# AegisIK/DistMLIP

Measured on NVIDIA H100. Metric: atoms/sec (energy+forces) CHGNet a-Si r_cut=5A, higher is better.
Workload: dtype f32

## Files before the change

### distmlip_b200/csrc/kernels.cu

```cuda
#include "atomic_virial.cuh"
#include "kernels.cuh"
#include "wgmma.cuh"

#include <algorithm>

namespace b2m {

std::atomic<long long> g_launch_count{0};

__device__ __forceinline__ float sigm(float x) {
  float e, r;
  asm("ex2.approx.ftz.f32 %0, %1;" : "=f"(e) : "f"(x * -1.4426950408889634f));
  asm("rcp.approx.ftz.f32 %0, %1;" : "=f"(r) : "f"(1.f + e));
  return r;
}
__device__ __forceinline__ float silu_f(float x) { return x * sigm(x); }
__device__ __forceinline__ float dsilu_f(float x) {
  float s = sigm(x);
  return s * (1.f + x * (1.f - s));
}

__device__ __forceinline__ uint32_t smem_u32(const void* p) { return (uint32_t)__cvta_generic_to_shared(p); }
__device__ __forceinline__ void mbar_init(uint64_t* bar, uint32_t count) {
  asm volatile("mbarrier.init.shared::cta.b64 [%0], %1;" ::"r"(smem_u32(bar)), "r"(count) : "memory");
}
__device__ __forceinline__ void fence_barrier_init() {
  asm volatile("fence.mbarrier_init.release.cluster;" ::: "memory");
  asm volatile("fence.proxy.async.shared::cta;" ::: "memory");
}
__device__ __forceinline__ void mbar_expect_tx(uint64_t* bar, uint32_t bytes) {
  asm volatile("mbarrier.arrive.expect_tx.shared::cta.b64 _, [%0], %1;" ::"r"(smem_u32(bar)), "r"(bytes) : "memory");
}
__device__ __forceinline__ void bulk_g2s(void* dst_smem, const void* src_gmem, uint32_t bytes, uint64_t* bar) {
  asm volatile("cp.async.bulk.shared::cluster.global.mbarrier::complete_tx::bytes [%0], [%1], %2, [%3];" ::"r"(
                   smem_u32(dst_smem)),
               "l"(src_gmem), "r"(bytes), "r"(smem_u32(bar))
               : "memory");
}
__device__ __forceinline__ void mbar_wait(uint64_t* bar, uint32_t parity) {
  uint32_t ok = 0;
  const uint32_t addr = smem_u32(bar);
  do {
    asm volatile(
        "{\n\t.reg .pred p;\n\tmbarrier.try_wait.parity.shared::cta.b64 p, [%1], %2;\n\tselp.u32 %0, 1, 0, p;\n\t}"
        : "=r"(ok)
        : "r"(addr), "r"(parity)
        : "memory");
  } while (!ok);
}
__device__ __forceinline__ uint32_t stage_parity(int it) { return (uint32_t)(it >> 1) & 1u; }
__device__ __forceinline__ void bulk_g2s_image(float* dst, const float* src, uint32_t bytes, uint64_t* bar) {
  mbar_expect_tx(bar, bytes);
  for (uint32_t o = 0; o < bytes; o += 16384u) bulk_g2s(dst + o / 4, src + o / 4, 16384u, bar);
}

__device__ __forceinline__ float ipowf(float x, int n) {
  float r = 1.f;
  for (int i = 0; i < n; i++) r *= x;
  return r;
}
__device__ __forceinline__ void rbf_env_k(float d, float freq, const RadialParams& rp, float& be, float& dbe) {
  const float invd = 1.f / d;
  const float w = freq / rp.rc;
  float s, c;
  sincosf(d * w, &s, &c);
  const float rbf = rp.norm * s * invd;
  const float drbf = rp.norm * (w * c * invd - s * invd * invd);
  const int p = rp.p;
  const float c1 = -(p + 1) * (p + 2) * 0.5f, c2 = (float)(p * (p + 2)), c3 = -p * (p + 1) * 0.5f;
  const float rho = rbf / rp.rc;
  const float rm1 = ipowf(rho, p - 1);
  const float r0 = rm1 * rho, r1 = r0 * rho, r2 = r1 * rho;
  const float env = 1.f + c1 * r0 + c2 * r1 + c3 * r2;
  const float denv = (c1 * p * rm1 + c2 * (p + 1) * r0 + c3 * (p + 2) * r1) / rp.rc;
  const bool ok = rbf <= rp.rc;
  be = ok ? env * rbf : 0.f;
  dbe = ok ? (env + rbf * denv) * drbf : 0.f;
}

constexpr int AR = 4, AC = 16;
struct Map {
  int branch, rb, cb;
  __device__ __forceinline__ Map() {
    const int tid = threadIdx.x;
    branch = tid >> 7;
    const int lane = tid & 31;
    rb = ((tid & 127) >> 5) * 16 + (lane >> 2);
    cb = 2 * (lane & 3);
  }
  __device__ __forceinline__ int row(int i) const { return 64 * (i >> 1) + rb + 8 * (i & 1); }
  __device__ __forceinline__ int col(int j) const { return 8 * (j >> 1) + cb + (j & 1); }
};

template <int KB>
__device__ __forceinline__ void wg_mma64(const float (&x)[KB][4], uint32_t b_hi, uint32_t b_lo, int bk, bool accumulate,
                                         float (&d)[32]) {
  constexpr uint32_t LBO = 8 * 128;
  uint32_t ah[KB][4], al[KB][4];
#pragma unroll
  for (int ks = 0; ks < KB; ks++)
#pragma unroll
    for (int q = 0; q < 4; q++) {
      ah[ks][q] = tf32_hi_bits(x[ks][q]);
      al[ks][q] = __float_as_uint(x[ks][q] - __uint_as_float(ah[ks][q]));
    }
  const uint32_t koff = (uint32_t)(bk / 4) * LBO;
  acc_fence(d);
  wgmma_fence();
#pragma unroll
  for (int ks = 0; ks < KB; ks++) {
#pragma unroll
    for (int term = 0; term < 3; term++) {
      const uint64_t bd = gmma_desc((term == 2 ? b_lo : b_hi) + koff + ks * 2 * LBO, LBO, 128u);
      wgmma_tf32_n64_rA(d, term == 1 ? al[ks] : ah[ks], bd, (accumulate || ks > 0 || term > 0) ? 1 : 0);
    }
  }
  wgmma_commit();
  wgmma_wait_all();
  acc_fence(d);
}

__device__ __forceinline__ void wg_mm64(const float* At, int lda, int row0, int acol, uint32_t b_hi, uint32_t b_lo,
                                        int bk, bool accumulate, float (&d)[32]) {
  const int lane = threadIdx.x & 31;
  const float* p0 = At + (row0 + ((threadIdx.x & 127) >> 5) * 16 + (lane >> 2)) * lda + acol + 2 * (lane & 3);
  const float* p1 = p0 + 8 * lda;
  float x[8][4];
#pragma unroll
  for (int ks = 0; ks < 8; ks++) {
    const float2 u = *reinterpret_cast<const float2*>(p0 + 8 * ks), v = *reinterpret_cast<const float2*>(p1 + 8 * ks);
    x[ks][0] = u.x, x[ks][1] = v.x, x[ks][2] = u.y, x[ks][3] = v.y;
  }
  wg_mma64(x, b_hi, b_lo, bk, accumulate, d);
}

__device__ __forceinline__ void gemm64(const float* At, int lda, int kofs, const float* Bcan, float (&acc)[AR][AC]) {
  const uint32_t bh = s_u32(Bcan), bl = bh + 4096u * 4u;
#pragma unroll
  for (int h = 0; h < 2; h++) {
    float d[32];
    wg_mm64(At, lda, 64 * h, kofs, bh, bl, 0, false, d);
#pragma unroll
    for (int q = 0; q < 32; q++) acc[2 * h + ((q >> 1) & 1)][2 * (q >> 2) + (q & 1)] = d[q];
  }
}

__device__ __forceinline__ void stage_w(float* Wsm, const float* __restrict__ g, int nfloat4) {
  for (int i = threadIdx.x; i < nfloat4; i += NT) reinterpret_cast<float4*>(Wsm)[i] = reinterpret_cast<const float4*>(g)[i];
  fence_proxy_async_smem();
}

__global__ void k_embed(int n, const int* __restrict__ type, const float* __restrict__ emb, float* __restrict__ x0) {
  const int64_t i = blockIdx.x * (int64_t)blockDim.x + threadIdx.x;
  if (i >= (int64_t)n * 16) return;
  const int r = (int)(i >> 4), c4 = (int)(i & 15);
  reinterpret_cast<float4*>(x0)[(size_t)r * 16 + c4] = reinterpret_cast<const float4*>(emb)[(size_t)type[r] * 16 + c4];
}
void launch_embed(cudaStream_t st, int n, const int* type, const float* emb, float* x0) {
  if (n <= 0) return;
  k_embed<<<cdiv((int64_t)n * 16, 256), 256, 0, st>>>(n, type, emb, x0);
  B2M_CK(cudaGetLastError());
  g_launch_count++;
}

__global__ void __launch_bounds__(256) k_bond_init(int nb, const float4* __restrict__ b_vec, RadialParams rp,
                                                   const float* __restrict__ W, float* __restrict__ out) {
  __shared__ float be_s[32][12];
  __shared__ float Ws[64 * 9];
  const int b0 = blockIdx.x * 32, tid = threadIdx.x;
  for (int i = tid; i < 576; i += 256) Ws[i] = W[i];
  for (int i = tid; i < 32 * 9; i += 256) {
    const int r = i / 9, k = i % 9;
    float be = 0.f, dbe;
    if (b0 + r < nb) rbf_env_k(b_vec[b0 + r].w, rp.freq[k], rp, be, dbe);
    be_s[r][k] = be;
  }
  __syncthreads();
  for (int i = tid; i < 32 * 64; i += 256) {
    const int r = i >> 6, c = i & 63;
    if (b0 + r >= nb) continue;
    float s = 0.f;
#pragma unroll
    for (int k = 0; k < 9; k++) s = fmaf(be_s[r][k], Ws[c * 9 + k], s);
    out[(size_t)(b0 + r) * 64 + c] = s;
  }
}
void launch_bond_init(cudaStream_t st, int nb, const float4* b_vec, RadialParams rp, const float* W, float* out) {
  if (nb <= 0) return;
  k_bond_init<<<cdiv(nb, 32), 256, 0, st>>>(nb, b_vec, rp, W, out);
  B2M_CK(cudaGetLastError());
  g_launch_count++;
}

struct AngleGeom {
  float cos_raw, cc, theta, na, nb;
  float va[3], vb[3];
};
__device__ __forceinline__ AngleGeom angle_geom(const float4 a, const float4 b) {
  AngleGeom g;
  g.va[0] = a.x, g.va[1] = a.y, g.va[2] = a.z;
  g.vb[0] = b.x, g.vb[1] = b.y, g.vb[2] = b.z;
  g.na = sqrtf(a.x * a.x + a.y * a.y + a.z * a.z);
  g.nb = sqrtf(b.x * b.x + b.y * b.y + b.z * b.z);
  g.cos_raw = -(a.x * b.x + a.y * b.y + a.z * b.z) / (g.na * g.nb);
  const float lo = -1.f + 1e-7f, hi = 1.f - 1e-7f;
  g.cc = fminf(fmaxf(g.cos_raw, lo), hi);
  g.theta = acosf(g.cc);
  return g;
}

__global__ void __launch_bounds__(256) k_angle_init(int64_t na, const int* __restrict__ a_in,
                                                    const int* __restrict__ a_out, const float4* __restrict__ b_vec,
                                                    const float* __restrict__ fa, const float* __restrict__ Wae,
                                                    float* __restrict__ ang0) {
  __shared__ float f_s[128][12];
  __shared__ float Ws[64 * 9];
  const int64_t r0 = (int64_t)blockIdx.x * 128;
  const int tid = threadIdx.x;
  for (int i = tid; i < 576; i += 256) Ws[i] = Wae[i];
  if (tid < 128) {
    const int64_t r = r0 + tid;
    if (r < na) {
      const AngleGeom g = angle_geom(b_vec[a_in[r]], b_vec[a_out[r]]);
      const float ipi = 0.318309886183790672f;
      for (int k = 0; k < 5; k++) {
        float s, c;
        sincosf(g.theta * fa[k], &s, &c);
        f_s[tid][2 * k] = c * ipi;
        if (k >= 1) f_s[tid][2 * k - 1] = s * ipi;
      }
    } else {
      for (int k = 0; k < 9; k++) f_s[tid][k] = 0.f;
    }
  }
  __syncthreads();
  for (int i = tid; i < 16 * 128; i += 256) {
    const int cq = i >> 7, r = i & 127;
    if (r0 + r >= na) continue;
    float v[4] = {0.f, 0.f, 0.f, 0.f};
#pragma unroll
    for (int k = 0; k < 9; k++) {
      const float f = f_s[r][k];
#pragma unroll
      for (int j = 0; j < 4; j++) v[j] = fmaf(f, Ws[(4 * cq + j) * 9 + k], v[j]);
    }
    *reinterpret_cast<float4*>(ang0 + (size_t)(r0 + r) * 64 + 4 * cq) = make_float4(v[0], v[1], v[2], v[3]);
  }
}
void launch_angle_init(cudaStream_t st, int64_t na, const int* a_in, const int* a_out, const float4* b_vec,
                       const float* fa, const float* Wae, float* ang0) {
  if (na <= 0) return;
  k_angle_init<<<cdiv(na, 128), 256, 0, st>>>(na, a_in, a_out, b_vec, fa, Wae, ang0);
  B2M_CK(cudaGetLastError());
  g_launch_count++;
}

__global__ void k_silu(int64_t n, const float* __restrict__ pre, float* __restrict__ out) {
  const int64_t i = blockIdx.x * (int64_t)blockDim.x + threadIdx.x;
  if (i < n) out[i] = silu_f(pre[i]);
}
__global__ void k_dsilu_mul(int64_t n, const float* __restrict__ pre, float* __restrict__ g) {
  const int64_t i = blockIdx.x * (int64_t)blockDim.x + threadIdx.x;
  if (i < n) g[i] *= dsilu_f(pre[i]);
}
void launch_silu(cudaStream_t st, int64_t n, const float* pre, float* out) {
  if (n <= 0) return;
  k_silu<<<cdiv(n, 256), 256, 0, st>>>(n, pre, out);
  B2M_CK(cudaGetLastError());
  g_launch_count++;
}
void launch_dsilu_mul(cudaStream_t st, int64_t n, const float* pre, float* g) {
  if (n <= 0) return;
  k_dsilu_mul<<<cdiv(n, 256), 256, 0, st>>>(n, pre, g);
  B2M_CK(cudaGetLastError());
  g_launch_count++;
}
void launch_zero_rows(cudaStream_t st, float* p, int64_t nfloats) {
  if (nfloats > 0) B2M_CK(cudaMemsetAsync(p, 0, nfloats * sizeof(float), st));
}

constexpr int LDE = 136;

struct EdgeRow {
  int src, dst, bond;
  float d;
};
__device__ __forceinline__ EdgeRow edge_row(const AtomConvArgs& a, int64_t e) {
  EdgeRow r{-1, -1, -1, 1.f};
  if (threadIdx.x < TM && e < a.E) {
    r.src = a.e_src[e];
    r.dst = a.e_dst[e];
    r.bond = a.e_bond[e];
    r.d = a.e_vec[e].w;
  }
  return r;
}
__device__ __forceinline__ void issue_gather(const AtomConvArgs& a, int64_t t, const EdgeRow& row, float* buf,
                                             uint64_t* bar, int* s_src, int* s_dst, int* s_bond, float* s_d) {
  const int tid = threadIdx.x;
  if (tid == 0) mbar_expect_tx(bar, (uint32_t)min((int64_t)TM, a.E - t * TM) * 512u);
  if (tid < TM) {
    if (s_src != nullptr) s_src[tid] = row.src;
    s_dst[tid] = row.dst;
    s_bond[tid] = row.bond;
    s_d[tid] = row.d;
    if (row.src >= 0) bulk_g2s(buf + tid * LDE, a.Aproj + (size_t)row.src * D2, 512u, bar);
  }
}
__device__ __forceinline__ void radial_rows(const AtomConvArgs& a, const float* s_d, int nvalid, float* be_s, float* be8,
                                            float* dbe_s, float* dbe8) {
  const int r = threadIdx.x & 127, half = threadIdx.x >> 7;
  const float d = s_d[r];
  const int k0 = half ? 5 : 0, k1 = half ? 9 : 5;
  for (int k = k0; k < k1; k++) {
    float be = 0.f, dbe = 0.f;
    if (r < nvalid) rbf_env_k(d, a.rp.freq[k], a.rp, be, dbe);
    *(k < 8 ? be_s + r * 8 + k : be8 + r) = be;
    if (dbe_s != nullptr) *(k < 8 ? dbe_s + r * 8 + k : dbe8 + r) = dbe;
  }
}
__device__ __forceinline__ float2 ld_f2(const float* p) { return *reinterpret_cast<const float2*>(p); }
__device__ __forceinline__ void st_f2(float* p, float x, float y) { *reinterpret_cast<float2*>(p) = make_float2(x, y); }

__device__ __forceinline__ constexpr int fq(int ii, int j) { return 4 * (j >> 1) + 2 * ii + (j & 1); }

__device__ __forceinline__ void radial_mma(const Map& m, int h, const float* x_s, const float* img, float (&d)[32]) {
  const float2 u = ld_f2(x_s + m.row(2 * h) * 8 + m.cb), v = ld_f2(x_s + m.row(2 * h + 1) * 8 + m.cb);
  const float x[1][4] = {{u.x, v.x, u.y, v.y}};
  uint32_t b = s_u32(img);
  asm volatile("" : "+r"(b));
  wg_mma64(x, b, b + 512u * 4u, 0, false, d);
}

__device__ __forceinline__ void first_layer_half(const AtomConvArgs& a, const Map& m, int h, const float* tile,
                                                 const int* s_dst, const int* s_bond, const float* be_s,
                                                 const float* be8, const float* rad, int nvalid,
                                                 float (&acc)[AR][AC]) {
  const int c0 = 64 * m.branch + m.cb;
  float2 cv[2][AC / 2], qv[2][AC / 2];
  float b8[2];
  bool viaQ[2], ok[2];
#pragma unroll
  for (int ii = 0; ii < 2; ii++) {
    const int r = m.row(2 * h + ii);
    const int dst = s_dst[r], bond = s_bond[r];
    ok[ii] = r < nvalid;
    viaQ[ii] = a.Qproj != nullptr && bond >= 0;
    const float* cp = a.Cproj + (size_t)max(dst, 0) * D2 + c0;
#pragma unroll
    for (int jj = 0; jj < AC / 2; jj++) cv[ii][jj] = dst >= 0 ? __ldg(reinterpret_cast<const float2*>(cp + 8 * jj)) : make_float2(0.f, 0.f);
    if (viaQ[ii]) {
      const float* qp = a.Qproj + (size_t)bond * D2 + c0;
#pragma unroll
      for (int jj = 0; jj < AC / 2; jj++) qv[ii][jj] = __ldg(reinterpret_cast<const float2*>(qp + 8 * jj));
    } else {
#pragma unroll
      for (int jj = 0; jj < AC / 2; jj++) qv[ii][jj] = make_float2(0.f, 0.f);
    }
    b8[ii] = be8[r];
  }
  float d[32];
  radial_mma(m, h, be_s, rad + ATOM_RAD_M + 1024 * m.branch, d);
#pragma unroll
  for (int j = 0; j < AC; j++) {
    const float m8 = rad[ATOM_RAD_M8 + 64 * m.branch + m.col(j)];
#pragma unroll
    for (int ii = 0; ii < 2; ii++) {
      const int r = m.row(2 * h + ii);
      const float x = tile[r * LDE + 64 * m.branch + m.col(j)];
      const float2 c2 = cv[ii][j >> 1], q2 = qv[ii][j >> 1];
      const float t = viaQ[ii] ? ((j & 1) ? q2.y : q2.x) : fmaf(b8[ii], m8, d[fq(ii, j)]);
      acc[2 * h + ii][j] = ok[ii] ? x + ((j & 1) ? c2.y : c2.x) + t : 0.f;
    }
  }
}

__device__ __forceinline__ void wg_mm64_acc(const float (&x)[AR][AC], int h, const float* Bcan, float (&acc)[AR][AC]) {
  float v[8][4];
#pragma unroll
  for (int ks = 0; ks < 8; ks++) {
    v[ks][0] = x[2 * h][2 * ks], v[ks][1] = x[2 * h + 1][2 * ks];
    v[ks][2] = x[2 * h][2 * ks + 1], v[ks][3] = x[2 * h + 1][2 * ks + 1];
  }
  const uint32_t b_hi = s_u32(Bcan);
  float d[32];
  wg_mma64(v, b_hi, b_hi + 4096u * 4u, 0, false, d);
#pragma unroll
  for (int q = 0; q < 32; q++) acc[2 * h + ((q >> 1) & 1)][2 * (q >> 2) + (q & 1)] = d[q];
}

__device__ __forceinline__ float quad_row_sum(const float (&v)[AR]) {
  const int l = threadIdx.x & 3;
  const bool b0 = l & 1, b1 = l & 2;
  float w[2];
#pragma unroll
  for (int h = 0; h < 2; h++)
    w[h] = (b0 ? v[2 * h + 1] : v[2 * h]) + __shfl_xor_sync(0xffffffffu, b0 ? v[2 * h] : v[2 * h + 1], 1);
  return (b1 ? w[1] : w[0]) + __shfl_xor_sync(0xffffffffu, b1 ? w[0] : w[1], 2);
}

__device__ __forceinline__ void red_add_v4(float* p, float4 v) {
  asm volatile("red.global.add.v4.f32 [%0], {%1, %2, %3, %4};" ::"l"(p), "f"(v.x), "f"(v.y), "f"(v.z), "f"(v.w)
               : "memory");
}

__device__ __forceinline__ void seg_add(float* out, int width, int col, int k, const float4& v, int& cur, float4& sum) {
  if (k != cur) {
    if (cur >= 0) red_add_v4(out + (size_t)cur * width + col, sum);
    cur = k;
    sum = make_float4(0.f, 0.f, 0.f, 0.f);
  }
  if (k >= 0) sum.x += v.x, sum.y += v.y, sum.z += v.z, sum.w += v.w;
}

template <int LPR>
__device__ __forceinline__ void scatter_rows(const float* tile, const int* key0, float* out0, const int* key1,
                                             float* out1, const int* gidx, float* gat, const int* sidx = nullptr,
                                             float* sto = nullptr) {
  constexpr int R = TM * LPR / NT, W = 4 * LPR, B = 8;
  static_assert(R % B == 0 && B % 4 == 0, "batches of B rows, their indices read as int4");
  const int q = threadIdx.x % LPR, r0 = threadIdx.x / LPR * R;
  float4 s0 = make_float4(0.f, 0.f, 0.f, 0.f), s1 = s0;
  int c0 = -1, c1 = -1;
#pragma unroll
  for (int b = 0; b < R; b += B) {
    float4 v[B];
    int k0[B], k1[B], kg[B], ks[B];
#pragma unroll
    for (int i = 0; i < B; i++) v[i] = *reinterpret_cast<const float4*>(tile + (r0 + b + i) * LDE + 4 * q);
    auto ld_idx = [&](const int* idx, bool on, int(&k)[B]) {
#pragma unroll
      for (int i = 0; i < B; i += 4) {
        const int4 x = on ? *reinterpret_cast<const int4*>(idx + r0 + b + i) : make_int4(-1, -1, -1, -1);
        k[i] = x.x, k[i + 1] = x.y, k[i + 2] = x.z, k[i + 3] = x.w;
      }
    };
    ld_idx(key0, out0 != nullptr, k0);
    ld_idx(key1, out1 != nullptr, k1);
    ld_idx(gidx, gat != nullptr, kg);
    ld_idx(sidx, sto != nullptr, ks);
#pragma unroll
    for (int i = 0; i < B; i++) {
      if (ks[i] >= 0) *reinterpret_cast<float4*>(sto + (size_t)ks[i] * W + 4 * q) = v[i];
      if (kg[i] >= 0) red_add_v4(gat + (size_t)kg[i] * W + 4 * q, v[i]);
      seg_add(out0, W, 4 * q, k0[i], v[i], c0, s0);
      seg_add(out1, W, 4 * q, k1[i], v[i], c1, s1);
    }
  }
  if (c0 >= 0) red_add_v4(out0 + (size_t)c0 * W + 4 * q, s0);
  if (c1 >= 0) red_add_v4(out1 + (size_t)c1 * W + 4 * q, s1);
}

struct AtomSmemFwd {
  static constexpr int kTile = 32;
  static constexpr int kW = kTile + 2 * TM * LDE;
  static constexpr int kRad = kW + 16384;
  static constexpr int kBe = kRad + ATOM_RAD;
  static constexpr int kBe8 = kBe + TM * 8;
  static constexpr int kB2 = kBe8 + TM;
  static constexpr int kD = kB2 + 128;
  static constexpr int kIdx = kD + 2 * TM;
  static constexpr int kTotal = kIdx + 4 * TM;
  static constexpr size_t bytes = (size_t)kTotal * 4;
};
static_assert(AtomSmemFwd::bytes <= 232448, "atom-conv forward shared memory");
static_assert(AtomSmemFwd::kW % 4 == 0 && AtomSmemFwd::kRad % 4 == 0 && AtomSmemFwd::kBe % 4 == 0,
              "16-byte aligned images and radial rows");

__global__ void __launch_bounds__(NT, 1) k_atomconv_fwd(const AtomConvArgs a) {
  extern __shared__ __align__(128) float smem[];
  uint64_t* mbar = reinterpret_cast<uint64_t*>(smem);
  float* Wsm = smem + AtomSmemFwd::kW;
  float* rad = smem + AtomSmemFwd::kRad;
  float* be_s = smem + AtomSmemFwd::kBe;
  float* be8 = smem + AtomSmemFwd::kBe8;
  float* b2s = smem + AtomSmemFwd::kB2;

  const int tid = threadIdx.x;
  const int64_t ntiles = (a.E + TM - 1) / TM, step = gridDim.x;
  auto tile_of = [&](int s) { return smem + AtomSmemFwd::kTile + s * TM * LDE; };
  auto d_of = [&](int s) { return smem + AtomSmemFwd::kD + s * TM; };
  auto dst_of = [&](int s) { return reinterpret_cast<int*>(smem + AtomSmemFwd::kIdx) + s * TM; };
  auto bond_of = [&](int s) { return reinterpret_cast<int*>(smem + AtomSmemFwd::kIdx) + (2 + s) * TM; };

  if (tid == 0) {
    mbar_init(&mbar[0], 1);
    mbar_init(&mbar[1], 1);
    fence_barrier_init();
  }
  EdgeRow nxt = edge_row(a, (int64_t)blockIdx.x * TM + tid);
  stage_w(Wsm, a.W2can, 4096);
  stage_w(rad, a.radial, ATOM_RAD / 4);
  if (tid < 128) b2s[tid] = a.b2[tid];
  __syncthreads();
  issue_gather(a, blockIdx.x, nxt, tile_of(0), &mbar[0], nullptr, dst_of(0), bond_of(0), d_of(0));
  nxt = edge_row(a, ((int64_t)blockIdx.x + step) * TM + tid);

  const Map m;
  int it = 0;
  for (int64_t t = blockIdx.x; t < ntiles; t += step, it++) {
    const int s = it & 1;
    float* tile = tile_of(s);
    const int* s_dst = dst_of(s);
    const int* s_bond = bond_of(s);
    const int nvalid = (int)min((int64_t)TM, a.E - t * TM);
    fence_proxy_async_smem();
    __syncthreads();
    if (t + step < ntiles) {
      issue_gather(a, t + step, nxt, tile_of(s ^ 1), &mbar[s ^ 1], nullptr, dst_of(s ^ 1), bond_of(s ^ 1), d_of(s ^ 1));
      nxt = edge_row(a, (t + 2 * step) * TM + tid);
    }
    radial_rows(a, d_of(s), nvalid, be_s, be8, nullptr, nullptr);
    mbar_wait(&mbar[s], stage_parity(it));
    __syncthreads();
    float acc[AR][AC];
#pragma unroll
    for (int h = 0; h < 2; h++) {
      first_layer_half(a, m, h, tile, s_dst, s_bond, be_s, be8, rad, nvalid, acc);
#pragma unroll
      for (int ii = 0; ii < 2; ii++)
#pragma unroll
        for (int j = 0; j < AC; j++) acc[2 * h + ii][j] = silu_f(acc[2 * h + ii][j]);
      wg_mm64_acc(acc, h, Wsm + m.branch * 8192, acc);
    }
#pragma unroll
    for (int i = 0; i < AR; i++)
#pragma unroll
      for (int j = 0; j < AC; j++) {
        const float u = acc[i][j] + b2s[m.branch * 64 + m.col(j)];
        acc[i][j] = m.branch == 0 ? silu_f(u) : sigm(u);
      }
    if (m.branch == 1) {
#pragma unroll
      for (int h = 0; h < 2; h++) {
        float w[32];
        radial_mma(m, h, be_s, rad + ATOM_RAD_WAB, w);
#pragma unroll
        for (int ii = 0; ii < 2; ii++) {
          const float b8 = be8[m.row(2 * h + ii)];
#pragma unroll
          for (int j = 0; j < AC; j++) acc[2 * h + ii][j] *= fmaf(b8, rad[ATOM_RAD_WAB8 + m.col(j)], w[fq(ii, j)]);
        }
      }
#pragma unroll
      for (int i = 0; i < AR; i++)
#pragma unroll
        for (int jj = 0; jj < AC / 2; jj++)
          st_f2(tile + m.row(i) * LDE + 64 + m.col(2 * jj), acc[i][2 * jj], acc[i][2 * jj + 1]);
    }
    __syncthreads();
    if (m.branch == 0) {
#pragma unroll
      for (int i = 0; i < AR; i++)
#pragma unroll
        for (int jj = 0; jj < AC / 2; jj++) {
          float* p = tile + m.row(i) * LDE + m.col(2 * jj);
          const float2 g = ld_f2(p + 64);
          st_f2(p, acc[i][2 * jj] * g.x, acc[i][2 * jj + 1] * g.y);
        }
    }
    __syncthreads();
    scatter_rows<16>(tile, s_dst, a.agg, nullptr, nullptr, nullptr, nullptr);
  }
}

void launch_atomconv_fwd(cudaStream_t st, const AtomConvArgs& a, int num_sms) {
  if (a.E <= 0) return;
  static PerDeviceOnce attr;
  if (auto once_ = attr.first(); once_) {
    B2M_CK(cudaFuncSetAttribute(k_atomconv_fwd, cudaFuncAttributeMaxDynamicSharedMemorySize, (int)AtomSmemFwd::bytes));
  }
  k_atomconv_fwd<<<std::min(cdiv(a.E, TM), num_sms), NT, AtomSmemFwd::bytes, st>>>(a);
  B2M_CK(cudaGetLastError());
  g_launch_count++;
}

struct AtomSmemBwd {
  static constexpr int kBuf = 32;
  static constexpr int kW = kBuf + 2 * TM * LDE;
  static constexpr int kRad = kW + 16384;
  static constexpr int kBe = kRad + ATOM_RAD;
  static constexpr int kDbe = kBe + TM * 8;
  static constexpr int kBe8 = kDbe + TM * 8;
  static constexpr int kDbe8 = kBe8 + TM;
  static constexpr int kB2 = kDbe8 + TM;
  static constexpr int kD = kB2 + 128;
  static constexpr int kIdx = kD + 2 * TM;
  static constexpr int kTotal = kIdx + 6 * TM;
  static constexpr size_t bytes = (size_t)kTotal * 4;
};
static_assert(AtomSmemBwd::bytes <= 232448, "atom-conv backward shared memory");
static_assert(AtomSmemBwd::kW % 4 == 0 && AtomSmemBwd::kRad % 4 == 0 && AtomSmemBwd::kBe % 4 == 0 &&
                  AtomSmemBwd::kDbe % 4 == 0,
              "16-byte aligned images and radial rows");

__global__ void __launch_bounds__(NT, 1) k_atomconv_bwd(const AtomConvArgs a) {
  extern __shared__ __align__(128) float smem[];
  uint64_t* gbar = reinterpret_cast<uint64_t*>(smem);
  uint64_t* wbar = gbar + 2;
  float* Wsm = smem + AtomSmemBwd::kW;
  float* rad_base = smem + AtomSmemBwd::kRad;
  float* be_s = smem + AtomSmemBwd::kBe;
  float* dbe_s = smem + AtomSmemBwd::kDbe;
  float* be8 = smem + AtomSmemBwd::kBe8;
  float* dbe8 = smem + AtomSmemBwd::kDbe8;
  float* b2s = smem + AtomSmemBwd::kB2;

  const int tid = threadIdx.x;
  const int64_t ntiles = (a.E + TM - 1) / TM, step = gridDim.x;
  const bool useQ = a.Qproj != nullptr;
  auto buf_of = [&](int s) { return smem + AtomSmemBwd::kBuf + s * TM * LDE; };
  auto d_of = [&](int s) { return smem + AtomSmemBwd::kD + s * TM; };
  auto src_of = [&](int s) { return reinterpret_cast<int*>(smem + AtomSmemBwd::kIdx) + s * TM; };
  auto dst_of = [&](int s) { return reinterpret_cast<int*>(smem + AtomSmemBwd::kIdx) + (2 + s) * TM; };
  auto bond_of = [&](int s) { return reinterpret_cast<int*>(smem + AtomSmemBwd::kIdx) + (4 + s) * TM; };

  if (tid == 0) {
    mbar_init(&gbar[0], 1);
    mbar_init(&gbar[1], 1);
    mbar_init(wbar, 1);
    fence_barrier_init();
  }
  EdgeRow nxt = edge_row(a, (int64_t)blockIdx.x * TM + tid);
  stage_w(rad_base, a.radial, ATOM_RAD / 4);
  if (tid < 128) b2s[tid] = a.b2[tid];
  __syncthreads();
  if (tid == 0) bulk_g2s_image(Wsm, a.W2can, 16384 * 4, wbar);
  issue_gather(a, blockIdx.x, nxt, buf_of(0), &gbar[0], src_of(0), dst_of(0), bond_of(0), d_of(0));
  nxt = edge_row(a, ((int64_t)blockIdx.x + step) * TM + tid);
  uint32_t wpar = 0;

  const Map m;
  const int c0 = 64 * m.branch;
  int it = 0;
  for (int64_t t = blockIdx.x; t < ntiles; t += step, it++) {
    float* rad = rad_base;
    asm volatile("" : "+l"(rad));
    const int s = it & 1;
    float* tileP = buf_of(s);
    float* tileH = buf_of(s ^ 1);
    const int* s_src = src_of(s);
    const int* s_dst = dst_of(s);
    const int* s_bond = bond_of(s);
    const int64_t e0 = t * TM;
    const int nvalid = (int)min((int64_t)TM, a.E - e0);
    __syncthreads();
    radial_rows(a, d_of(s), nvalid, be_s, be8, dbe_s, dbe8);
    mbar_wait(&gbar[s], stage_parity(it));
    mbar_wait(wbar, wpar);
    wpar ^= 1;
    __syncthreads();
    float acc[AR][AC];
#pragma unroll
    for (int h = 0; h < 2; h++) {
      first_layer_half(a, m, h, tileP, s_dst, s_bond, be_s, be8, rad, nvalid, acc);
#pragma unroll
      for (int ii = 0; ii < 2; ii++)
#pragma unroll
        for (int jj = 0; jj < AC / 2; jj++) {
          float* p = tileP + m.row(2 * h + ii) * LDE + c0 + m.col(2 * jj);
          float& x0 = acc[2 * h + ii][2 * jj];
          float& x1 = acc[2 * h + ii][2 * jj + 1];
          st_f2(p, x0, x1);
          x0 = silu_f(x0);
          x1 = silu_f(x1);
        }
      wg_mm64_acc(acc, h, Wsm + m.branch * 8192, acc);
#pragma unroll
      for (int ii = 0; ii < 2; ii++)
#pragma unroll
        for (int jj = 0; jj < AC / 2; jj++) {
          const float u0 = acc[2 * h + ii][2 * jj] + b2s[m.branch * 64 + m.col(2 * jj)];
          const float u1 = acc[2 * h + ii][2 * jj + 1] + b2s[m.branch * 64 + m.col(2 * jj + 1)];
          st_f2(tileH + m.row(2 * h + ii) * LDE + c0 + m.col(2 * jj), m.branch == 0 ? u0 : sigm(u0),
                m.branch == 0 ? u1 : sigm(u1));
        }
    }
    __syncthreads();
    if (tid == 0) bulk_g2s_image(Wsm, a.W2Tcan, 16384 * 4, wbar);
    float sd[AR];
#pragma unroll
    for (int h = 0; h < 2; h++) {
      int dst[2];
      float2 gm2[2][AC / 2];
#pragma unroll
      for (int ii = 0; ii < 2; ii++) {
        dst[ii] = s_dst[m.row(2 * h + ii)];
        const float* gp = a.gagg + (size_t)max(dst[ii], 0) * D + m.cb;
#pragma unroll
        for (int jj = 0; jj < AC / 2; jj++)
          gm2[ii][jj] = dst[ii] >= 0 ? __ldg(reinterpret_cast<const float2*>(gp + 8 * jj)) : make_float2(0.f, 0.f);
      }
      float w[32];
      radial_mma(m, h, be_s, rad + ATOM_RAD_WAB, w);
#pragma unroll
      for (int ii = 0; ii < 2; ii++) {
        const int i = 2 * h + ii;
        const int r = m.row(i);
        const float b8 = be8[r];
#pragma unroll
        for (int jj = 0; jj < AC / 2; jj++) {
          const float2 ow2 = ld_f2(tileH + r * LDE + c0 + m.col(2 * jj));
          const float2 pt2 = ld_f2(tileH + r * LDE + (64 - c0) + m.col(2 * jj));
          const float2 wk2 = ld_f2(rad + ATOM_RAD_WAB8 + m.col(2 * jj));
#pragma unroll
          for (int e = 0; e < 2; e++) {
            const int j = 2 * jj + e;
            const float x = e ? ow2.y : ow2.x;
            const float pt = e ? pt2.y : pt2.x;
            const float gm = e ? gm2[ii][jj].y : gm2[ii][jj].x;
            const float wab = fmaf(b8, e ? wk2.y : wk2.x, w[fq(ii, j)]);
            float g = 0.f, gwv = 0.f;
            if (dst[ii] >= 0) {
              if (m.branch == 0) {
                const float sg = sigm(x);
                const float oL = x * sg;
                gwv = gm * oL * pt;
                g = gm * pt * wab * (sg * (1.f + x * (1.f - sg)));
              } else {
                const float oL = silu_f(pt);
                g = gm * oL * wab * x * (1.f - x);
              }
            }
            acc[i][j] = g;
            w[fq(ii, j)] = gwv;
          }
        }
      }
      sd[2 * h] = sd[2 * h + 1] = 0.f;
      if (m.branch == 0) {
        float dw[32];
        radial_mma(m, h, dbe_s, rad + ATOM_RAD_WAB, dw);
#pragma unroll
        for (int ii = 0; ii < 2; ii++) {
          const float db8 = dbe8[m.row(2 * h + ii)];
#pragma unroll
          for (int j = 0; j < AC; j++)
            sd[2 * h + ii] = fmaf(w[fq(ii, j)], fmaf(db8, rad[ATOM_RAD_WAB8 + m.col(j)], dw[fq(ii, j)]), sd[2 * h + ii]);
        }
      }
      if (h == 0) mbar_wait(wbar, wpar);
      wg_mm64_acc(acc, h, Wsm + m.branch * 8192, acc);
#pragma unroll
      for (int ii = 0; ii < 2; ii++)
#pragma unroll
        for (int jj = 0; jj < AC / 2; jj++) {
          float* p = tileP + m.row(2 * h + ii) * LDE + c0 + m.col(2 * jj);
          const float2 pre = ld_f2(p);
          float& x0 = acc[2 * h + ii][2 * jj];
          float& x1 = acc[2 * h + ii][2 * jj + 1];
          x0 *= dsilu_f(pre.x);
          x1 *= dsilu_f(pre.y);
          st_f2(p, x0, x1);
        }
      float dm[32];
      radial_mma(m, h, dbe_s, rad + ATOM_RAD_M + 1024 * m.branch, dm);
#pragma unroll
      for (int ii = 0; ii < 2; ii++) {
        const int r = m.row(2 * h + ii);
        const float db8 = dbe8[r];
        float s = 0.f;
#pragma unroll
        for (int jj = 0; jj < AC / 2; jj++) {
          const float2 mk = ld_f2(rad + ATOM_RAD_M8 + c0 + m.col(2 * jj));
          s = fmaf(acc[2 * h + ii][2 * jj], fmaf(db8, mk.x, dm[fq(ii, 2 * jj)]), s);
          s = fmaf(acc[2 * h + ii][2 * jj + 1], fmaf(db8, mk.y, dm[fq(ii, 2 * jj + 1)]), s);
        }
        if (r < nvalid && !(useQ && s_bond[r] >= 0)) sd[2 * h + ii] += s;
      }
    }
    wpar ^= 1;
    fence_proxy_async_smem();
    __syncthreads();
    if (t + step < ntiles) {
      if (tid == 0) bulk_g2s_image(Wsm, a.W2can, 16384 * 4, wbar);
      issue_gather(a, t + step, nxt, tileH, &gbar[s ^ 1], src_of(s ^ 1), dst_of(s ^ 1), bond_of(s ^ 1), d_of(s ^ 1));
      nxt = edge_row(a, (t + 2 * step) * TM + tid);
    }
    {
      const float v = quad_row_sum(sd);
      const int r = m.row(tid & 3);
      if (m.branch == 1) be8[r] = v;
      __syncthreads();
      if (m.branch == 0 && r < nvalid) a.gd[e0 + r] += v + be8[r];
    }
    scatter_rows<32>(tileP, s_dst, a.gA != nullptr ? a.gC : nullptr, nullptr, nullptr, s_src, a.gA, s_bond,
                     useQ ? a.gQ : nullptr);
  }
}

void launch_atomconv_bwd(cudaStream_t st, const AtomConvArgs& a, int num_sms) {
  if (a.E <= 0) return;
  static PerDeviceOnce attr;
  if (auto once_ = attr.first(); once_) {
    B2M_CK(cudaFuncSetAttribute(k_atomconv_bwd, cudaFuncAttributeMaxDynamicSharedMemorySize, (int)AtomSmemBwd::bytes));
  }
  k_atomconv_bwd<<<std::min(cdiv(a.E, TM), num_sms), NT, AtomSmemBwd::bytes, st>>>(a);
  B2M_CK(cudaGetLastError());
  g_launch_count++;
}

struct LineSmem {
  static constexpr int kBuf = 32;
  static constexpr int kW = kBuf + 2 * TM * LDE;
  static constexpr int kB2 = kW + 16384;
  static constexpr int kIdx = kB2 + 128;
  static constexpr int kTotal = kIdx + 6 * TM;
  static constexpr size_t bytes = (size_t)kTotal * 4;
};
static_assert(LineSmem::bytes <= 232448, "line-graph shared memory");

struct LineSm {
  float* smem;
  __device__ __forceinline__ uint64_t* hbar() const { return reinterpret_cast<uint64_t*>(smem); }
  __device__ __forceinline__ uint64_t* abar() const { return hbar() + 2; }
  __device__ __forceinline__ uint64_t* wbar() const { return hbar() + 4; }
  __device__ __forceinline__ float* buf(int s) const { return smem + LineSmem::kBuf + s * TM * LDE; }
  __device__ __forceinline__ float* W() const { return smem + LineSmem::kW; }
  __device__ __forceinline__ float* b2() const { return smem + LineSmem::kB2; }
  __device__ __forceinline__ int* idx(int s, int k) const {
    return reinterpret_cast<int*>(smem + LineSmem::kIdx) + (2 * k + s) * TM;
  }
};

struct AngleIdx {
  int a, b, c;
};
__device__ __forceinline__ AngleIdx angle_idx(const LineArgs& a, int64_t r) {
  AngleIdx x{-1, -1, -1};
  if (threadIdx.x < TM && r < a.A) {
    x.a = a.a_in[r];
    x.b = a.a_out[r];
    x.c = a.a_ctr[r];
  }
  return x;
}
__device__ __forceinline__ void line_issue_ha(const LineArgs& a, const LineSm& sm, int64_t t, const AngleIdx& x,
                                             float* buf, int s) {
  const int tid = threadIdx.x;
  if (tid == 0) mbar_expect_tx(&sm.hbar()[s], (uint32_t)min((int64_t)TM, a.A - t * TM) * 512u);
  if (tid < TM) {
    sm.idx(s, 0)[tid] = x.a;
    sm.idx(s, 1)[tid] = x.b;
    sm.idx(s, 2)[tid] = x.c;
    if (x.a >= 0) bulk_g2s(buf + tid * LDE, a.Ha + (size_t)x.a * D2, 512u, &sm.hbar()[s]);
  }
}
__device__ __forceinline__ void line_issue_ang(const LineArgs& a, const LineSm& sm, int64_t t, float* buf, int s) {
  const int tid = threadIdx.x;
  const int nvalid = (int)min((int64_t)TM, a.A - t * TM);
  if (tid == 0) mbar_expect_tx(&sm.abar()[s], (uint32_t)nvalid * 256u);
  if (tid < nvalid) bulk_g2s(buf + tid * LDE + 64, a.ang + (size_t)(t * TM + tid) * D, 256u, &sm.abar()[s]);
}
__device__ __forceinline__ AngleIdx line_prologue(const LineArgs& a, const LineSm& sm) {
  const int tid = threadIdx.x;
  if (tid == 0) {
    for (int i = 0; i < 5; i++) mbar_init(&sm.hbar()[i], 1);
    fence_barrier_init();
  }
  AngleIdx x = angle_idx(a, (int64_t)blockIdx.x * TM + tid);
  if (tid < 128) sm.b2()[tid] = a.b2 ? a.b2[tid] : 0.f;
  __syncthreads();
  if (tid == 0) bulk_g2s_image(sm.W(), a.Wgcan, 16384 * 4, sm.wbar());
  line_issue_ha(a, sm, blockIdx.x, x, sm.buf(0), 0);
  line_issue_ang(a, sm, blockIdx.x, sm.buf(1), 0);
  return angle_idx(a, ((int64_t)blockIdx.x + gridDim.x) * TM + tid);
}

__device__ __forceinline__ void line_first_layer(const LineArgs& a, const Map& m, const float* P, const int* s_b,
                                                 const int* s_c, int nvalid, float (&acc)[AR][AC]) {
  const int c0 = 64 * m.branch + m.cb;
#pragma unroll
  for (int i = 0; i < AR; i++) {
    const int r = m.row(i);
    const bool ok = r < nvalid;
    const float* hb = a.Hb + (size_t)(ok ? s_b[r] : 0) * D2 + c0;
    const float* xc = a.Xc + (size_t)(ok ? s_c[r] : 0) * D2 + c0;
    float2 hv[AC / 2], xv[AC / 2];
#pragma unroll
    for (int jj = 0; jj < AC / 2; jj++) {
      hv[jj] = ok ? __ldg(reinterpret_cast<const float2*>(hb + 8 * jj)) : make_float2(0.f, 0.f);
      xv[jj] = ok ? __ldg(reinterpret_cast<const float2*>(xc + 8 * jj)) : make_float2(0.f, 0.f);
    }
#pragma unroll
    for (int jj = 0; jj < AC / 2; jj++) {
      const float2 ha = ok ? ld_f2(P + r * LDE + c0 + 8 * jj) : make_float2(0.f, 0.f);
      float& x0 = acc[i][2 * jj];
      float& x1 = acc[i][2 * jj + 1];
      x0 = ok ? ha.x + x0 + hv[jj].x + xv[jj].x : 0.f;
      x1 = ok ? ha.y + x1 + hv[jj].y + xv[jj].y : 0.f;
    }
  }
}

__device__ __forceinline__ void red_add_v2(float* p, float x, float y) {
  asm volatile("red.global.add.v2.f32 [%0], {%1, %2};" ::"l"(p), "f"(x), "f"(y) : "memory");
}

template <bool HIDDEN>
__global__ void __launch_bounds__(NT, 1) k_line_fwd(const LineArgs a) {
  extern __shared__ __align__(128) float smem[];
  const LineSm sm{smem};
  const float* b2s = sm.b2();
  const int tid = threadIdx.x;
  const int64_t ntiles = (a.A + TM - 1) / TM, step = gridDim.x;
  AngleIdx nxt = line_prologue(a, sm);
  uint32_t wpar = 0;

  int it = 0;
  for (int64_t t = blockIdx.x; t < ntiles; t += step, it++) {
    const int s = it & 1;
    float* P = sm.buf(s);
    float* Q = sm.buf(s ^ 1);
    const int* s_b = sm.idx(s, 1);
    const int* s_c = sm.idx(s, 2);
    const int64_t r0 = t * TM;
    const int nvalid = (int)min((int64_t)TM, a.A - r0);
    const bool more = t + step < ntiles;
    const Map m;
    float acc[AR][AC];
    mbar_wait(&sm.abar()[s], stage_parity(it));
    mbar_wait(sm.wbar(), wpar);
    if (HIDDEN) wpar ^= 1;
    gemm64(Q, LDE, 64, sm.W() + m.branch * 8192, acc);
    fence_proxy_async_smem();
    __syncthreads();
    if (more) {
      line_issue_ha(a, sm, t + step, nxt, Q, s ^ 1);
      nxt = angle_idx(a, (t + 2 * step) * TM + tid);
    }
// ... 631 lines not shown
```

Measured before the change: 2.243 million.

## Split atom-conv forward into three independent warpgroups with 64-edge tiles

The atom-conv forward kernel is rebuilt so each block runs three independent 128-thread warpgroups. Each warpgroup owns its own 64-edge tile, mbarrier and named barrier, and computes both the core and gate branches itself, so the branches no longer exchange data through shared memory. Block-wide __syncthreads and the double-buffered gather are replaced by per-warpgroup bar.sync, which lets the warpgroups drift apart and overlap each other's gather latency. In exchange each warpgroup has a single tile buffer, so its own gather is no longer prefetched during compute, and the smaller tiles mean more scatter atomics per edge.

```diff
diff --git a/distmlip_b200/csrc/kernels.cu b/distmlip_b200/csrc/kernels.cu
--- a/distmlip_b200/csrc/kernels.cu
+++ b/distmlip_b200/csrc/kernels.cu
@@ -145,8 +145,9 @@
   }
 }
 
+template <int NTH = NT>
 __device__ __forceinline__ void stage_w(float* Wsm, const float* __restrict__ g, int nfloat4) {
-  for (int i = threadIdx.x; i < nfloat4; i += NT) reinterpret_cast<float4*>(Wsm)[i] = reinterpret_cast<const float4*>(g)[i];
+  for (int i = threadIdx.x; i < nfloat4; i += NTH) reinterpret_cast<float4*>(Wsm)[i] = reinterpret_cast<const float4*>(g)[i];
   fence_proxy_async_smem();
 }
 
@@ -285,9 +286,9 @@
   int src, dst, bond;
   float d;
 };
-__device__ __forceinline__ EdgeRow edge_row(const AtomConvArgs& a, int64_t e) {
+__device__ __forceinline__ EdgeRow edge_row(const AtomConvArgs& a, int64_t e, bool has_row) {
   EdgeRow r{-1, -1, -1, 1.f};
-  if (threadIdx.x < TM && e < a.E) {
+  if (has_row && e < a.E) {
     r.src = a.e_src[e];
     r.dst = a.e_dst[e];
     r.bond = a.e_bond[e];
@@ -295,21 +296,22 @@
   }
   return r;
 }
-__device__ __forceinline__ void issue_gather(const AtomConvArgs& a, int64_t t, const EdgeRow& row, float* buf,
+template <int ROWS>
+__device__ __forceinline__ void issue_gather(const AtomConvArgs& a, int64_t t, const EdgeRow& row, int lr, float* buf,
                                              uint64_t* bar, int* s_src, int* s_dst, int* s_bond, float* s_d) {
-  const int tid = threadIdx.x;
-  if (tid == 0) mbar_expect_tx(bar, (uint32_t)min((int64_t)TM, a.E - t * TM) * 512u);
-  if (tid < TM) {
-    if (s_src != nullptr) s_src[tid] = row.src;
-    s_dst[tid] = row.dst;
-    s_bond[tid] = row.bond;
-    s_d[tid] = row.d;
-    if (row.src >= 0) bulk_g2s(buf + tid * LDE, a.Aproj + (size_t)row.src * D2, 512u, bar);
-  }
-}
+  if (lr == 0) mbar_expect_tx(bar, (uint32_t)min((int64_t)ROWS, a.E - t * ROWS) * 512u);
+  if (lr < ROWS) {
+    if (s_src != nullptr) s_src[lr] = row.src;
+    s_dst[lr] = row.dst;
+    s_bond[lr] = row.bond;
+    s_d[lr] = row.d;
+    if (row.src >= 0) bulk_g2s(buf + lr * LDE, a.Aproj + (size_t)row.src * D2, 512u, bar);
+  }
+}
+template <int ROWS>
 __device__ __forceinline__ void radial_rows(const AtomConvArgs& a, const float* s_d, int nvalid, float* be_s, float* be8,
                                             float* dbe_s, float* dbe8) {
-  const int r = threadIdx.x & 127, half = threadIdx.x >> 7;
+  const int r = threadIdx.x % ROWS, half = (threadIdx.x / ROWS) & 1;
   const float d = s_d[r];
   const int k0 = half ? 5 : 0, k1 = half ? 9 : 5;
   for (int k = k0; k < k1; k++) {
@@ -332,10 +334,11 @@
   wg_mma64(x, b, b + 512u * 4u, 0, false, d);
 }
 
+template <int R>
 __device__ __forceinline__ void first_layer_half(const AtomConvArgs& a, const Map& m, int h, const float* tile,
                                                  const int* s_dst, const int* s_bond, const float* be_s,
                                                  const float* be8, const float* rad, int nvalid,
-                                                 float (&acc)[AR][AC]) {
+                                                 float (&acc)[R][AC]) {
   const int c0 = 64 * m.branch + m.cb;
   float2 cv[2][AC / 2], qv[2][AC / 2];
   float b8[2];
@@ -375,7 +378,8 @@
   }
 }
 
-__device__ __forceinline__ void wg_mm64_acc(const float (&x)[AR][AC], int h, const float* Bcan, float (&acc)[AR][AC]) {
+template <int R>
+__device__ __forceinline__ void wg_mm64_acc(const float (&x)[R][AC], int h, const float* Bcan, float (&acc)[R][AC]) {
   float v[8][4];
 #pragma unroll
   for (int ks = 0; ks < 8; ks++) {
@@ -413,13 +417,13 @@
   if (k >= 0) sum.x += v.x, sum.y += v.y, sum.z += v.z, sum.w += v.w;
 }
 
-template <int LPR>
+template <int LPR, int ROWS = TM, int NTH = NT>
 __device__ __forceinline__ void scatter_rows(const float* tile, const int* key0, float* out0, const int* key1,
                                              float* out1, const int* gidx, float* gat, const int* sidx = nullptr,
                                              float* sto = nullptr) {
-  constexpr int R = TM * LPR / NT, W = 4 * LPR, B = 8;
+  constexpr int R = ROWS * LPR / NTH, W = 4 * LPR, B = 8;
   static_assert(R % B == 0 && B % 4 == 0, "batches of B rows, their indices read as int4");
-  const int q = threadIdx.x % LPR, r0 = threadIdx.x / LPR * R;
+  const int t = threadIdx.x % NTH, q = t % LPR, r0 = t / LPR * R;
   float4 s0 = make_float4(0.f, 0.f, 0.f, 0.f), s1 = s0;
   int c0 = -1, c1 = -1;
 #pragma unroll
@@ -451,116 +455,107 @@
   if (c1 >= 0) red_add_v4(out1 + (size_t)c1 * W + 4 * q, s1);
 }
 
+constexpr int TW = 64;
+constexpr int WGF = 3, NTF = 128 * WGF;
 struct AtomSmemFwd {
   static constexpr int kTile = 32;
-  static constexpr int kW = kTile + 2 * TM * LDE;
+  static constexpr int kW = kTile + WGF * TW * LDE;
   static constexpr int kRad = kW + 16384;
   static constexpr int kBe = kRad + ATOM_RAD;
-  static constexpr int kBe8 = kBe + TM * 8;
-  static constexpr int kB2 = kBe8 + TM;
+  static constexpr int kBe8 = kBe + WGF * TW * 8;
+  static constexpr int kB2 = kBe8 + WGF * TW;
   static constexpr int kD = kB2 + 128;
-  static constexpr int kIdx = kD + 2 * TM;
-  static constexpr int kTotal = kIdx + 4 * TM;
+  static constexpr int kIdx = kD + WGF * TW;
+  static constexpr int kTotal = kIdx + 2 * WGF * TW;
   static constexpr size_t bytes = (size_t)kTotal * 4;
 };
 static_assert(AtomSmemFwd::bytes <= 232448, "atom-conv forward shared memory");
-static_assert(AtomSmemFwd::kW % 4 == 0 && AtomSmemFwd::kRad % 4 == 0 && AtomSmemFwd::kBe % 4 == 0,
-              "16-byte aligned images and radial rows");
-
-__global__ void __launch_bounds__(NT, 1) k_atomconv_fwd(const AtomConvArgs a) {
+static_assert(AtomSmemFwd::kW % 4 == 0 && AtomSmemFwd::kRad % 4 == 0 && AtomSmemFwd::kBe % 4 == 0 &&
+                  AtomSmemFwd::kIdx % 4 == 0,
+              "16-byte aligned images, radial rows and index slots");
+
+__device__ __forceinline__ void wg_sync(int w) { asm volatile("bar.sync %0, 128;" ::"r"(1 + w) : "memory"); }
+
+__global__ void __launch_bounds__(NTF, 1) k_atomconv_fwd(const AtomConvArgs a) {
   extern __shared__ __align__(128) float smem[];
-  uint64_t* mbar = reinterpret_cast<uint64_t*>(smem);
-  float* Wsm = smem + AtomSmemFwd::kW;
-  float* rad = smem + AtomSmemFwd::kRad;
-  float* be_s = smem + AtomSmemFwd::kBe;
-  float* be8 = smem + AtomSmemFwd::kBe8;
-  float* b2s = smem + AtomSmemFwd::kB2;
-
-  const int tid = threadIdx.x;
-  const int64_t ntiles = (a.E + TM - 1) / TM, step = gridDim.x;
-  auto tile_of = [&](int s) { return smem + AtomSmemFwd::kTile + s * TM * LDE; };
-  auto d_of = [&](int s) { return smem + AtomSmemFwd::kD + s * TM; };
-  auto dst_of = [&](int s) { return reinterpret_cast<int*>(smem + AtomSmemFwd::kIdx) + s * TM; };
-  auto bond_of = [&](int s) { return reinterpret_cast<int*>(smem + AtomSmemFwd::kIdx) + (2 + s) * TM; };
-
+  const int tid = threadIdx.x, w = tid >> 7, lr = tid & 127;
+  uint64_t* mbar = reinterpret_cast<uint64_t*>(smem) + w;
+  const float* Wsm = smem + AtomSmemFwd::kW;
+  const float* rad = smem + AtomSmemFwd::kRad;
+  const float* b2s = smem + AtomSmemFwd::kB2;
+  float* tile = smem + AtomSmemFwd::kTile + w * TW * LDE;
+  float* be_s = smem + AtomSmemFwd::kBe + w * TW * 8;
+  float* be8 = smem + AtomSmemFwd::kBe8 + w * TW;
+  float* s_d = smem + AtomSmemFwd::kD + w * TW;
+  int* s_dst = reinterpret_cast<int*>(smem + AtomSmemFwd::kIdx) + w * TW;
+  int* s_bond = reinterpret_cast<int*>(smem + AtomSmemFwd::kIdx) + (WGF + w) * TW;
+
+  const int64_t ntiles = (a.E + TW - 1) / TW, first = WGF * (int64_t)blockIdx.x + w, step = WGF * (int64_t)gridDim.x;
   if (tid == 0) {
-    mbar_init(&mbar[0], 1);
-    mbar_init(&mbar[1], 1);
+    for (int i = 0; i < WGF; i++) mbar_init(reinterpret_cast<uint64_t*>(smem) + i, 1);
     fence_barrier_init();
   }
-  EdgeRow nxt = edge_row(a, (int64_t)blockIdx.x * TM + tid);
-  stage_w(Wsm, a.W2can, 4096);
-  stage_w(rad, a.radial, ATOM_RAD / 4);
-  if (tid < 128) b2s[tid] = a.b2[tid];
+  EdgeRow nxt = edge_row(a, first * TW + lr, lr < TW);
+  stage_w<NTF>(smem + AtomSmemFwd::kW, a.W2can, 4096);
+  stage_w<NTF>(smem + AtomSmemFwd::kRad, a.radial, ATOM_RAD / 4);
+  if (tid < 128) smem[AtomSmemFwd::kB2 + tid] = a.b2[tid];
   __syncthreads();
-  issue_gather(a, blockIdx.x, nxt, tile_of(0), &mbar[0], nullptr, dst_of(0), bond_of(0), d_of(0));
-  nxt = edge_row(a, ((int64_t)blockIdx.x + step) * TM + tid);
+  if (first < ntiles)
+    issue_gather<TW>(a, first, nxt, lr, tile, mbar, nullptr, s_dst, s_bond, s_d);
+  nxt = edge_row(a, (first + step) * TW + lr, lr < TW);
 
   const Map m;
+  Map mL = m, mG = m;
+  mL.branch = 0;
+  mG.branch = 1;
   int it = 0;
-  for (int64_t t = blockIdx.x; t < ntiles; t += step, it++) {
-    const int s = it & 1;
-    float* tile = tile_of(s);
-    const int* s_dst = dst_of(s);
-    const int* s_bond = bond_of(s);
-    const int nvalid = (int)min((int64_t)TM, a.E - t * TM);
+  for (int64_t t = first; t < ntiles; t += step, it++) {
+    const int nvalid = (int)min((int64_t)TW, a.E - t * TW);
+    wg_sync(w);
+    radial_rows<TW>(a, s_d, nvalid, be_s, be8, nullptr, nullptr);
+    mbar_wait(mbar, (uint32_t)it & 1u);
+    wg_sync(w);
+    float L[2][AC];
+    first_layer_half(a, mL, 0, tile, s_dst, s_bond, be_s, be8, rad, nvalid, L);
+#pragma unroll
+    for (int ii = 0; ii < 2; ii++)
+#pragma unroll
+      for (int j = 0; j < AC; j++) L[ii][j] = silu_f(L[ii][j]);
+    wg_mm64_acc(L, 0, Wsm, L);
+#pragma unroll
+    for (int ii = 0; ii < 2; ii++)
+#pragma unroll
+      for (int j = 0; j < AC; j++) L[ii][j] = silu_f(L[ii][j] + b2s[m.col(j)]);
+    float G[2][AC];
+    first_layer_half(a, mG, 0, tile, s_dst, s_bond, be_s, be8, rad, nvalid, G);
+#pragma unroll
+    for (int ii = 0; ii < 2; ii++)
+#pragma unroll
+      for (int j = 0; j < AC; j++) G[ii][j] = silu_f(G[ii][j]);
+    wg_mm64_acc(G, 0, Wsm + 8192, G);
+    float wab[32];
+    radial_mma(m, 0, be_s, rad + ATOM_RAD_WAB, wab);
+#pragma unroll
+    for (int ii = 0; ii < 2; ii++) {
+      const int r = m.row(ii);
+      const float b8 = be8[r];
+      float mv[AC];
+#pragma unroll
+      for (int j = 0; j < AC; j++) {
+        const float g = sigm(G[ii][j] + b2s[64 + m.col(j)]) * fmaf(b8, rad[ATOM_RAD_WAB8 + m.col(j)], wab[fq(ii, j)]);
+        mv[j] = L[ii][j] * g;
+      }
+#pragma unroll
+      for (int jj = 0; jj < AC / 2; jj++) st_f2(tile + r * LDE + m.col(2 * jj), mv[2 * jj], mv[2 * jj + 1]);
+    }
+    wg_sync(w);
+    scatter_rows<16, TW, 128>(tile, s_dst, a.agg, nullptr, nullptr, nullptr, nullptr);
     fence_proxy_async_smem();
-    __syncthreads();
+    wg_sync(w);
     if (t + step < ntiles) {
-      issue_gather(a, t + step, nxt, tile_of(s ^ 1), &mbar[s ^ 1], nullptr, dst_of(s ^ 1), bond_of(s ^ 1), d_of(s ^ 1));
-      nxt = edge_row(a, (t + 2 * step) * TM + tid);
-    }
-    radial_rows(a, d_of(s), nvalid, be_s, be8, nullptr, nullptr);
-    mbar_wait(&mbar[s], stage_parity(it));
-    __syncthreads();
-    float acc[AR][AC];
-#pragma unroll
-    for (int h = 0; h < 2; h++) {
-      first_layer_half(a, m, h, tile, s_dst, s_bond, be_s, be8, rad, nvalid, acc);
-#pragma unroll
-      for (int ii = 0; ii < 2; ii++)
-#pragma unroll
-        for (int j = 0; j < AC; j++) acc[2 * h + ii][j] = silu_f(acc[2 * h + ii][j]);
-      wg_mm64_acc(acc, h, Wsm + m.branch * 8192, acc);
-    }
-#pragma unroll
-    for (int i = 0; i < AR; i++)
-#pragma unroll
-      for (int j = 0; j < AC; j++) {
-        const float u = acc[i][j] + b2s[m.branch * 64 + m.col(j)];
-        acc[i][j] = m.branch == 0 ? silu_f(u) : sigm(u);
-      }
-    if (m.branch == 1) {
-#pragma unroll
-      for (int h = 0; h < 2; h++) {
-        float w[32];
-        radial_mma(m, h, be_s, rad + ATOM_RAD_WAB, w);
-#pragma unroll
-        for (int ii = 0; ii < 2; ii++) {
-          const float b8 = be8[m.row(2 * h + ii)];
-#pragma unroll
-          for (int j = 0; j < AC; j++) acc[2 * h + ii][j] *= fmaf(b8, rad[ATOM_RAD_WAB8 + m.col(j)], w[fq(ii, j)]);
-        }
-      }
-#pragma unroll
-      for (int i = 0; i < AR; i++)
-#pragma unroll
-        for (int jj = 0; jj < AC / 2; jj++)
-          st_f2(tile + m.row(i) * LDE + 64 + m.col(2 * jj), acc[i][2 * jj], acc[i][2 * jj + 1]);
-    }
-    __syncthreads();
-    if (m.branch == 0) {
-#pragma unroll
-      for (int i = 0; i < AR; i++)
-#pragma unroll
-        for (int jj = 0; jj < AC / 2; jj++) {
-          float* p = tile + m.row(i) * LDE + m.col(2 * jj);
-          const float2 g = ld_f2(p + 64);
-          st_f2(p, acc[i][2 * jj] * g.x, acc[i][2 * jj + 1] * g.y);
-        }
-    }
-    __syncthreads();
-    scatter_rows<16>(tile, s_dst, a.agg, nullptr, nullptr, nullptr, nullptr);
+      issue_gather<TW>(a, t + step, nxt, lr, tile, mbar, nullptr, s_dst, s_bond, s_d);
+      nxt = edge_row(a, (t + 2 * step) * TW + lr, lr < TW);
+    }
   }
 }
 
@@ -570,7 +565,7 @@
   if (auto once_ = attr.first(); once_) {
     B2M_CK(cudaFuncSetAttribute(k_atomconv_fwd, cudaFuncAttributeMaxDynamicSharedMemorySize, (int)AtomSmemFwd::bytes));
   }
-  k_atomconv_fwd<<<std::min(cdiv(a.E, TM), num_sms), NT, AtomSmemFwd::bytes, st>>>(a);
+  k_atomconv_fwd<<<std::min(cdiv(cdiv(a.E, TW), WGF), num_sms), NTF, AtomSmemFwd::bytes, st>>>(a);
   B2M_CK(cudaGetLastError());
   g_launch_count++;
 }
@@ -621,13 +616,13 @@
     mbar_init(wbar, 1);
     fence_barrier_init();
   }
-  EdgeRow nxt = edge_row(a, (int64_t)blockIdx.x * TM + tid);
+  EdgeRow nxt = edge_row(a, (int64_t)blockIdx.x * TM + tid, threadIdx.x < TM);
   stage_w(rad_base, a.radial, ATOM_RAD / 4);
   if (tid < 128) b2s[tid] = a.b2[tid];
   __syncthreads();
   if (tid == 0) bulk_g2s_image(Wsm, a.W2can, 16384 * 4, wbar);
-  issue_gather(a, blockIdx.x, nxt, buf_of(0), &gbar[0], src_of(0), dst_of(0), bond_of(0), d_of(0));
-  nxt = edge_row(a, ((int64_t)blockIdx.x + step) * TM + tid);
+  issue_gather<TM>(a, blockIdx.x, nxt, tid, buf_of(0), &gbar[0], src_of(0), dst_of(0), bond_of(0), d_of(0));
+  nxt = edge_row(a, ((int64_t)blockIdx.x + step) * TM + tid, threadIdx.x < TM);
   uint32_t wpar = 0;
 
   const Map m;
@@ -645,7 +640,7 @@
     const int64_t e0 = t * TM;
     const int nvalid = (int)min((int64_t)TM, a.E - e0);
     __syncthreads();
-    radial_rows(a, d_of(s), nvalid, be_s, be8, dbe_s, dbe8);
+    radial_rows<TM>(a, d_of(s), nvalid, be_s, be8, dbe_s, dbe8);
     mbar_wait(&gbar[s], stage_parity(it));
     mbar_wait(wbar, wpar);
     wpar ^= 1;
@@ -774,8 +769,8 @@
     __syncthreads();
     if (t + step < ntiles) {
       if (tid == 0) bulk_g2s_image(Wsm, a.W2can, 16384 * 4, wbar);
-      issue_gather(a, t + step, nxt, tileH, &gbar[s ^ 1], src_of(s ^ 1), dst_of(s ^ 1), bond_of(s ^ 1), d_of(s ^ 1));
-      nxt = edge_row(a, (t + 2 * step) * TM + tid);
+      issue_gather<TM>(a, t + step, nxt, tid, tileH, &gbar[s ^ 1], src_of(s ^ 1), dst_of(s ^ 1), bond_of(s ^ 1), d_of(s ^ 1));
+      nxt = edge_row(a, (t + 2 * step) * TM + tid, threadIdx.x < TM);
     }
     {
       const float v = quad_row_sum(sd);
```

After: 2.352 million, median of 6. 1.05x the previous value.
